# laboroai/border

Measured on AMD Instinct MI355X. Metric: agent opt-steps/sec (DQN Atari 84x84x4, batch 256), higher is better.
Workload: dtype f32 (conv2 / conv3 forward: 3xbf16 operand split, 6 products)

## Files before the change

border_amd/csrc/dqn.hip:

```cpp
#include <algorithm>
#include <atomic>
#include <chrono>
#include <cmath>
#include <string>

#include "common.hpp"
#include "agent_base.hpp"
#include "igemm.hpp"
#include "conv1_bf16_img.hpp"
#include "cnn_layers.hpp"
#include "igemm_b3.hpp"
#include "act_small.hpp"
#include "dqn_rollback.hpp"

using namespace bdr;

namespace {

#ifndef BDR_TEAMS
#define BDR_TEAMS 2
#endif
#ifndef BDR_TEAMS_FWD_C3
#define BDR_TEAMS_FWD_C3 BDR_TEAMS
#endif
#ifndef BDR_TEAMS_DX_L1
#define BDR_TEAMS_DX_L1 BDR_TEAMS
#endif
#ifndef BDR_TEAMS_DX_C3
#define BDR_TEAMS_DX_C3 BDR_TEAMS
#endif
#ifndef BDR_TEAMS_FWD_L1
#define BDR_TEAMS_FWD_L1 1
#endif
#ifndef BDR_TEAMS_FWD_C2
#define BDR_TEAMS_FWD_C2 1
#endif
#ifndef BDR_TEAMS_DX_C2
#define BDR_TEAMS_DX_C2 1
#endif
#ifndef BDR_TAIL_OVERLAP
#define BDR_TAIL_OVERLAP 1
#endif
#ifndef BDR_DXC2_MERGED
#define BDR_DXC2_MERGED 2
#endif
#ifndef BDR_FWDC3_SHAPE
#define BDR_FWDC3_SHAPE 1, 2, 1, 1
#endif
using FwdC3D = FwdConvP<GeomC3, BDR_FWDC3_SHAPE>;
constexpr size_t PL2_U16 = (size_t)3 * 64 * 512, PL3_U16 = (size_t)3 * 64 * 576;
constexpr size_t CPL_W2 = 0, CPL_W3 = PL2_U16, CPL_U16 = PL2_U16 + PL3_U16;
__device__ __forceinline__ size_t cpl_index(int k, int n) { return ((size_t)(k >> 5) * 64 + n) * 32 + (k & 31); }

__device__ __forceinline__ void conv_plane_store(uint16_t* __restrict__ pl, int layer, int e, float x)
{
    uint16_t v[3];
    split3_rn(x, v);
    const size_t n = (size_t)(layer ? 576 : 512) * 64, o = cpl_index(e >> 6, e & 63);
    uint16_t* d = pl + (layer ? CPL_W3 : CPL_W2);
    d[o] = v[0]; d[n + o] = v[1]; d[2 * n + o] = v[2];
}

__global__ __launch_bounds__(256) void k_conv_planes(const float* __restrict__ w2, const float* __restrict__ w3, uint16_t* __restrict__ pl)
{
    const int i = blockIdx.x * 256 + threadIdx.x;
    if (i < 512 * 64) conv_plane_store(pl, 0, i, w2[i]);
    else if (i < 512 * 64 + 576 * 64) conv_plane_store(pl, 1, i - 512 * 64, w3[i - 512 * 64]);
}
#ifndef BDR_FWDC2_B3_SHAPE
#define BDR_FWDC2_B3_SHAPE 2, 2
#endif
#ifndef BDR_FWDC3_B3_SHAPE
#define BDR_FWDC3_B3_SHAPE 2, 2
#endif
struct FwdB3Args : FwdArgs { const uint16_t* wpl[MAXZ]; };
template <class G, int WM_, int WN_, int TM_ = 1, int TN_ = 1>
struct FwdB3 : FwdP<G, AFwd<G>, WM_, WN_, false, 0, TM_, TN_> {
    using Args = FwdB3Args;
    __device__ static const uint4* b_chunk(const Args& a, int z, int, int pl, int kt, int n, int kq)
    {
        return reinterpret_cast<const uint4*>(a.wpl[z] + (size_t)pl * G::COUT * G::K + cpl_index(kt * 32 + kq * 8, n));
    }
};
using FwdC2B3 = FwdB3<GeomC2, BDR_FWDC2_B3_SHAPE>;
using FwdC3B3 = FwdB3<GeomC3, BDR_FWDC3_B3_SHAPE>;
constexpr int TEAMS_FWD_C2 = BDR_TEAMS_FWD_C2, TEAMS_FWD_C3 = BDR_TEAMS_FWD_C3, TEAMS_FWD_L1 = BDR_TEAMS_FWD_L1, TEAMS_DX_L1 = BDR_TEAMS_DX_L1,
              TEAMS_DX_C3 = BDR_TEAMS_DX_C3, TEAMS_DX_C2 = BDR_TEAMS_DX_C2;

struct HeadArgs {
    const float* p1[MAXZ];
    const float* b4[MAXZ];
    const float* w5[MAXZ];
    const float* b5[MAXZ];
    float* h1[MAXZ];
    float* q[MAXZ];
    int B, A, S;
};

struct TdArgs {
    int double_dqn;
    const uint8_t* act;
    int act_bytes;
    const float* reward;
    const int8_t* term;
    float* dh1;
    float* dq;
    float* pred;
    float* tgt;
    float* loss_row;
    int B, A;
    float gamma;
    int loss_kind;
    const float* weight;
    float* td_abs;
    int has_clip; float clip_min, clip_max;
    unsigned* err;
    const float* q_tgt_mem;
    int z_tgt, z_sel;
    unsigned* wait_sig; unsigned wait_epoch; unsigned long long wait_limit; unsigned* sig_err;
};

constexpr int HEAD_ROWS = 2;
template <int S, int AMAX>
__global__ __launch_bounds__(64 * HEAD_ROWS * MAXZ) void k_head(HeadArgs a, TdArgs t, int nz, int td)
{
    __shared__ float sq[HEAD_ROWS][MAXZ][64];
    const int lane = threadIdx.x & 63, wave = __builtin_amdgcn_readfirstlane(threadIdx.x >> 6);
    const int r = wave / nz, z = wave % nz;
    const int row = blockIdx.x * HEAD_ROWS + r;
    const bool valid = row < a.B;
    const int rw = valid ? row : 0;
    const int A = a.A;
    f32x4 part[S][2];
#pragma unroll
    for (int s = 0; s < S; ++s) {
        const float* p = a.p1[z] + ((size_t)s * a.B + rw) * 512 + lane * 8;
        part[s][0] = *reinterpret_cast<const f32x4*>(p);
        part[s][1] = *reinterpret_cast<const f32x4*>(p + 4);
    }
    const f32x4 b4lo = *reinterpret_cast<const f32x4*>(a.b4[z] + lane * 8), b4hi = *reinterpret_cast<const f32x4*>(a.b4[z] + lane * 8 + 4);
    const float* w5 = a.w5[z] + lane * 8;
    float wreg[8][AMAX];
#pragma unroll
    for (int k = 0; k < AMAX; ++k) {
        const float* wk = w5 + (size_t)min(k, A - 1) * 512;
        const f32x4 lo = *reinterpret_cast<const f32x4*>(wk), hi = *reinterpret_cast<const f32x4*>(wk + 4);
#pragma unroll
        for (int j = 0; j < 4; ++j) { wreg[j][k] = lo[j]; wreg[4 + j][k] = hi[j]; }
    }
    const float b5 = lane < A ? a.b5[z][lane] : 0.f;
    long long act = 0; float reward = 0.f, wgt = 1.f; int term = 0;
    if (td && z == 0) {
        act = *reinterpret_cast<const long long*>(t.act + (size_t)rw * t.act_bytes);
        if (act < 0 || act >= A) {
            if (lane == 0 && t.err) atomicOr(t.err + bdr_agent::ERR_ACTION, 1u);
            act = act < 0 ? 0 : A - 1;
        }
        reward = t.reward[rw]; term = (int)t.term[rw];
        if (t.weight) wgt = t.weight[rw];
    }

    f32x4 h[2] = {f32x4{0, 0, 0, 0}, f32x4{0, 0, 0, 0}};
#pragma unroll
    for (int s = 0; s < S; ++s) { h[0] += part[s][0]; h[1] += part[s][1]; }
    float hv[8];
#pragma unroll
    for (int j = 0; j < 8; ++j) {
        const float v = h[j >> 2][j & 3] + (j < 4 ? b4lo[j & 3] : b4hi[j & 3]);
        hv[j] = v > 0.f ? v : 0.f;
    }
    asm volatile("" ::"v"(act), "v"(reward), "v"(term), "v"(wgt), "v"(b5));
    if (valid) {
        float* ho = a.h1[z] + (size_t)row * 512 + lane * 8;
        *reinterpret_cast<f32x4*>(ho) = f32x4{hv[0], hv[1], hv[2], hv[3]};
        *reinterpret_cast<f32x4*>(ho + 4) = f32x4{hv[4], hv[5], hv[6], hv[7]};
    }
    float sk[AMAX];
#pragma unroll
    for (int k = 0; k < AMAX; ++k) {
        float s = 0.f;
#pragma unroll
        for (int j = 0; j < 8; ++j) s = fmaf(hv[j], wreg[j][k], s);
        sk[k] = s;
    }
#pragma unroll
    for (int off = 32; off > 0; off >>= 1)
#pragma unroll
        for (int k = 0; k < AMAX; ++k) sk[k] += __shfl_xor(sk[k], off);
    float qv = 0.f;
#pragma unroll
    for (int k = 0; k < AMAX; ++k) qv = lane == k ? sk[k] : qv;
    qv += b5;
    if (lane < A) {
        if (valid) a.q[z][(size_t)row * A + lane] = qv;
        sq[r][z][lane] = qv;
    }
    if (!td) return;
    if (t.q_tgt_mem && t.wait_sig) {
        if (threadIdx.x == 0) {
            const unsigned long long t0 = wall_clock64();
            while ((int)(__hip_atomic_load(t.wait_sig, __ATOMIC_ACQUIRE, __HIP_MEMORY_SCOPE_AGENT) - t.wait_epoch) < 0) {
                __builtin_amdgcn_s_sleep(2);
                if (__hip_atomic_load(t.sig_err, __ATOMIC_RELAXED, __HIP_MEMORY_SCOPE_AGENT) != 0) break;
                if (wall_clock64() - t0 > t.wait_limit) {
                    __hip_atomic_store(t.sig_err, 100u, __ATOMIC_RELAXED, __HIP_MEMORY_SCOPE_AGENT);
                    if (t.err) __hip_atomic_store(t.err + bdr_agent::ERR_GATE, 100u, __ATOMIC_RELAXED, __HIP_MEMORY_SCOPE_AGENT);
                    break;
                }
            }
        }
    }
    __syncthreads();
    if (z != 0 || !valid) return;
    if (t.q_tgt_mem) {
        __builtin_amdgcn_fence(__ATOMIC_ACQUIRE, "agent");
        if (lane < A) sq[r][MAXZ - 1][lane] = __builtin_nontemporal_load(t.q_tgt_mem + (size_t)row * A + lane);
    }
    const float* q_tg = t.q_tgt_mem ? sq[r][MAXZ - 1] : sq[r][t.z_tgt];
    const float* sel = t.z_sel >= 0 ? sq[r][t.z_sel] : q_tg;
    float v = lane < A ? sel[lane] : -INFINITY;
    int idx = lane;
#pragma unroll
    for (int off = 32; off > 0; off >>= 1) {
        const float ov = __shfl_xor(v, off);
        const int oi = __shfl_xor(idx, off);
        if (ov > v || (ov == v && oi < idx)) { v = ov; idx = oi; }
    }
    const float qn = q_tg[idx];
    const float pred = sq[r][0][act];
    const float tgt = td_target(reward, (float)(1 - term), t.gamma, qn);
    const TdLossIn li{t.loss_kind, t.weight != nullptr, wgt, t.has_clip, t.clip_min, t.clip_max};
    float lossb, tdv;
    const float dl = td_loss_row(pred, tgt, li, lossb, tdv);
    const float dq = dl / (float)a.B;
    if (lane == 0) {
        t.dq[row] = dq; t.pred[row] = pred; t.tgt[row] = tgt; t.loss_row[row] = lossb;
        if (t.td_abs) t.td_abs[row] = tdv;
    }
// ... 196 lines not shown
    BDR_TRY(alloc_f(&a->a1_alt, (size_t)B * 400 * 32));
    BDR_TRY(alloc_f(&a->dh1, (size_t)B * 512));
    BDR_TRY(alloc_f(&a->dy3, (size_t)B * 49 * 64));
    BDR_TRY(alloc_f(&a->dy2, (size_t)B * 81 * 64));
    BDR_TRY(alloc_f(&a->dy1, (size_t)B * 400 * 32));
    BDR_TRY(alloc_f(&a->dq, B)); BDR_TRY(alloc_f(&a->pred, B)); BDR_TRY(alloc_f(&a->tgt, B));
    BDR_TRY(alloc_f(&a->loss_row, B));
    const DwPlan p = dw_plan(B, a->ar.ns);
    BDR_TRY(alloc_f(&a->part, p.total));
    a->part_floats = p.total;
    a->B = B;
    return BDR_OK;
}

struct ConvReduceAdamArgs {
    Reduce3Args r;
    float* p; const float* g; float* m; float* v;
    float* gbase;
    size_t rest0_4, n4;
    AdamScalars s;
    int reduce_blocks;
    const unsigned* poison;
    int reduce_only;
    unsigned long long* applied; unsigned long long step;
    unsigned long long* applied2;
    int wg_base;
    uint16_t* cpl;
};
constexpr int SIG_HEAD = 0, SIG_DXL1 = 1, SIG_DXC3 = 2, SIG_SIDE = 3, SIG_GATHER = 4, SIG_TEST = 5, SIG_TEST_ERR = 6, SIG_ERR = 7, SIG_TGT = 8, SIG_TRACK = 9, SIG_MAIN_END = 10, SIG_XCONV = 11, SIG_XFC = 14;
constexpr int SIG_DXC2 = 15, SIG_CONV23 = SIG_SIDE;
__global__ __launch_bounds__(64) void k_gate(unsigned* sig, int which, unsigned epoch, unsigned long long* waited, int publish,
                                             unsigned long long limit = 1000000000ull , int err_slot = SIG_ERR,
                                             unsigned* dev_err = nullptr)
{
    if (threadIdx.x != 0) return;
    if (publish >= 0) __hip_atomic_store(sig + publish, epoch, __ATOMIC_RELAXED, __HIP_MEMORY_SCOPE_AGENT);
    if (err_slot == SIG_ERR && __hip_atomic_load(sig + SIG_ERR, __ATOMIC_RELAXED, __HIP_MEMORY_SCOPE_AGENT) != 0) return;
    const unsigned long long t0 = wall_clock64();
    while ((int)(__hip_atomic_load(sig + which, __ATOMIC_ACQUIRE, __HIP_MEMORY_SCOPE_AGENT) - epoch) < 0) {
        __builtin_amdgcn_s_sleep(4);
        if (wall_clock64() - t0 > limit || (err_slot == SIG_ERR && __hip_atomic_load(sig + SIG_ERR, __ATOMIC_RELAXED, __HIP_MEMORY_SCOPE_AGENT) != 0)) {
            __hip_atomic_store(sig + err_slot, 1u + (unsigned)which, __ATOMIC_RELAXED, __HIP_MEMORY_SCOPE_AGENT);
            if (dev_err) __hip_atomic_store(dev_err + bdr_agent::ERR_GATE, 1u + (unsigned)which, __ATOMIC_RELAXED, __HIP_MEMORY_SCOPE_AGENT);
            return;
        }
    }
    if (waited) {
        const unsigned long long dt = wall_clock64() - t0;
        waited[0] += dt; waited[1] += 1;
        unsigned long long* mx = waited + 22 - (which == SIG_SIDE ? 4 : which);
        if (dt > *mx) *mx = dt;
        if (which == SIG_SIDE) {
            const unsigned long long ts = *reinterpret_cast<volatile unsigned long long*>(sig + 12);
            if (ts && t0 > ts) waited[12] += t0 - ts;
        }
    }
}
__global__ __launch_bounds__(64) void k_signal(unsigned* sig, int which, unsigned epoch)
{
    if (threadIdx.x == 0 && which == SIG_SIDE) *reinterpret_cast<volatile unsigned long long*>(sig + 12) = wall_clock64();
    if (threadIdx.x == 0) __hip_atomic_store(sig + which, epoch, __ATOMIC_RELAXED, __HIP_MEMORY_SCOPE_AGENT);
}

__global__ void k_copy_word_unless(unsigned long long* dst, const unsigned long long* src, const unsigned* poison) { if (!(poison && *poison)) *dst = *src; }

__global__ __launch_bounds__(256) void k_reduce_adam(ConvReduceAdamArgs a)
{
    const bool poisoned = a.reduce_only || (a.poison && *a.poison != 0);
    if (a.applied && !poisoned && blockIdx.x == 0 && threadIdx.x == 0) { *a.applied = a.step; if (a.applied2) *a.applied2 = a.step; }
    if ((int)blockIdx.x >= a.reduce_blocks) {
        if (poisoned) return;
        const size_t i = a.rest0_4 + (size_t)(blockIdx.x - a.reduce_blocks) * 256 + threadIdx.x;
        if (i >= a.n4) return;
        f32x4 pp = reinterpret_cast<f32x4*>(a.p)[i], gg = reinterpret_cast<const f32x4*>(a.g)[i];
        f32x4 mm = reinterpret_cast<f32x4*>(a.m)[i], vv = reinterpret_cast<f32x4*>(a.v)[i];
#pragma unroll
        for (int j = 0; j < 4; ++j) {
            float pe = pp[j], me = mm[j], ve = vv[j];
            adam_element(pe, gg[j], me, ve, a.s);
            pp[j] = pe; mm[j] = me; vv[j] = ve;
        }
        reinterpret_cast<f32x4*>(a.p)[i] = pp;
        reinterpret_cast<f32x4*>(a.m)[i] = mm;
        reinterpret_cast<f32x4*>(a.v)[i] = vv;
        return;
    }
    __shared__ float red[8][32];
    const int bx = (int)blockIdx.x + a.wg_base;
    const int s_id = bx >= a.r.seg[2].wg0 ? 2 : (bx >= a.r.seg[1].wg0 ? 1 : 0);
    const ReduceSeg& sg = a.r.seg[s_id];
    const int o = threadIdx.x & 31, grp = threadIdx.x >> 5;
    const int i = (bx - sg.wg0) * 32 + o;
    float s = 0.f;
    if (i < sg.n) {
        int c = grp;
        for (; c + 24 < sg.chunks; c += 32) {
            const float v0 = sg.part[(size_t)c * sg.stride + i], v1 = sg.part[(size_t)(c + 8) * sg.stride + i];
            const float v2 = sg.part[(size_t)(c + 16) * sg.stride + i], v3 = sg.part[(size_t)(c + 24) * sg.stride + i];
            s += v0; s += v1; s += v2; s += v3;
        }
        for (; c < sg.chunks; c += 8) s += sg.part[(size_t)c * sg.stride + i];
    }
    red[grp][o] = s;
    __syncthreads();
    if (grp == 0 && i < sg.n) {
        float t = red[0][o];
#pragma unroll
        for (int k = 1; k < 8; ++k) t += red[k][o];
        const float g = i < sg.n_weights ? t * sg.wscale : t;
        sg.g[i] = g;
        if (poisoned) return;
        const size_t e = (size_t)(sg.g - a.gbase) + i;
        float pe = a.p[e], me = a.m[e], ve = a.v[e];
        adam_element(pe, g, me, ve, a.s);
        a.p[e] = pe; a.m[e] = me; a.v[e] = ve;
        if (a.cpl && s_id >= 1 && i < sg.n_weights) conv_plane_store(a.cpl, s_id - 1, i, pe);
    }
}

int effective_sched(DqnCnn* a);

struct NetInst { const uint8_t* x; const float* params; int slot; };

int32_t forward(DqnCnn* a, const NetInst* inst, int nz, int B, const TdArgs* td = nullptr, hipStream_t st = nullptr)
{
    if (!st) st = a->stream;
    const Arena& ar = a->ar;
    FwdArgs f{};
    bool uses_q = false;
    for (int z = 0; z < nz; ++z) uses_q = uses_q || inst[z].params == a->q;
    if (uses_q) BDR_TRY(a->join_exchange(true, false));
    {
        Conv1Args c{};
        c.M = B * 400; c.nz = nz;
        for (int z = 0; z < nz; ++z) {
            c.x[z] = inst[z].x; c.w1[z] = inst[z].params + ar.w1; c.bias[z] = inst[z].params + ar.b1; c.out[z] = a->a1[inst[z].slot];
        }
        Bracket br(a, "fwd_conv1");
        BDR_HIP(conv1_forward(ar.ns, B, st, c));
    }
    if (uses_q && st == a->stream) BDR_TRY(a->join_conv23());
    f.M = B * 81;
    for (int z = 0; z < nz; ++z) { f.x[z] = a->a1[inst[z].slot]; f.w[z] = inst[z].params + ar.w2; f.bias[z] = inst[z].params + ar.b2; f.out[z] = a->a2[inst[z].slot]; }
    bool b3 = a->conv_b3;
    FwdB3Args fb{};
    for (int z = 0; z < nz && b3; ++z) b3 = inst[z].params == a->q || inst[z].params == a->q_tgt;
    for (int z = 0; z < nz && b3; ++z) {
        const int set = inst[z].params == a->q ? 0 : 1;
        if (a->cpl_fresh[set] && !a->cpl_escaped[set]) continue;
        hipLaunchKernelGGL(k_conv_planes, dim3((512 * 64 + 576 * 64 + 255) / 256), dim3(256), 0, st, inst[z].params + ar.w2, inst[z].params + ar.w3, a->cpl[set]);
        BDR_HIP(hipGetLastError());
        a->cpl_fresh[set] = true;
    }
    if (b3) {
        static_cast<FwdArgs&>(fb) = f;
        for (int z = 0; z < nz; ++z) fb.wpl[z] = a->cpl[inst[z].params == a->q ? 0 : 1] + CPL_W2;
        Bracket br(a, "fwd_conv2");
        BDR_HIP((launch_igemm_b3<FwdC2B3, 6>(st, dim3(m_tiles<FwdC2B3>(f.M) * n_tiles<FwdC2B3>(), 1, nz), fb)));
    } else { Bracket br(a, "fwd_conv2"); BDR_HIP((launch_igemm<FwdC2, TEAMS_FWD_C2>(st, dim3(m_tiles<FwdC2>(f.M) * n_tiles<FwdC2>(), 1, nz), f))); }
    f.M = B * 49;
    for (int z = 0; z < nz; ++z) { f.x[z] = a->a2[inst[z].slot]; f.w[z] = inst[z].params + ar.w3; f.bias[z] = inst[z].params + ar.b3; f.out[z] = a->a3[inst[z].slot]; }
    if (b3) {
        static_cast<FwdArgs&>(fb) = f;
        for (int z = 0; z < nz; ++z) fb.wpl[z] = a->cpl[inst[z].params == a->q ? 0 : 1] + CPL_W3;
        Bracket br(a, "fwd_conv3");
        BDR_HIP((launch_igemm_b3<FwdC3B3, 6>(st, dim3(m_tiles<FwdC3B3>(f.M) * n_tiles<FwdC3B3>(), 1, nz), fb)));
    } else { Bracket br(a, "fwd_conv3"); BDR_HIP((launch_igemm<FwdC3D, TEAMS_FWD_C3>(st, dim3(m_tiles<FwdC3D>(f.M) * n_tiles<FwdC3D>(), 1, nz), f))); }
    f.M = B; f.nkt_per_split = (98 + L1_SPLIT - 1) / L1_SPLIT;
    for (int z = 0; z < nz; ++z) { f.x[z] = a->a3[inst[z].slot]; f.w[z] = inst[z].params + ar.w4; f.bias[z] = nullptr; f.out[z] = a->p1[inst[z].slot]; }
    if (uses_q) BDR_TRY(a->join_exchange(false, true));
    {
        Bracket br(a, "fwd_l1");
#if BDR_L1_XSPLIT
        static_assert(L1_SPLIT == 8, "FwdL1X: one k-slice per XCD");
        BDR_HIP((launch_igemm<FwdL1X, TEAMS_FWD_L1>(st, dim3(m_tiles<FwdL1X>(B) * n_tiles<FwdL1X>() * 8, 1, nz), f)));
#else
        if (nz % 2 == 0) BDR_HIP((launch_igemm<FwdL1Z2, TEAMS_FWD_L1>(st, dim3(((B + 63) / 64) * 16, L1_SPLIT, nz / 2), f)));
        else BDR_HIP((launch_igemm<FwdL1, TEAMS_FWD_L1>(st, dim3(((B + 63) / 64) * 8, L1_SPLIT, nz), f)));
#endif
    }
    HeadArgs h{};
    h.B = B; h.A = ar.A; h.S = L1_SPLIT;
    for (int z = 0; z < nz; ++z) {
        h.p1[z] = a->p1[inst[z].slot]; h.b4[z] = inst[z].params + ar.b4; h.w5[z] = inst[z].params + ar.w5;
        h.b5[z] = inst[z].params + ar.b5; h.h1[z] = a->h1[inst[z].slot]; h.q[z] = a->qv[inst[z].slot];
    }
    {
        Bracket br(a, td ? "head_fwd_td" : "head_fwd");
        const dim3 grid((B + HEAD_ROWS - 1) / HEAD_ROWS), block(64 * HEAD_ROWS * nz);
        const TdArgs tv = td ? *td : TdArgs{};
        hipEvent_t stop = td && effective_sched(a) == 1 && a->kev ? a->ev_fork[0] : nullptr;
        const int tdi = td ? 1 : 0;
        if (ar.A <= 8) hipExtLaunchKernelGGL((k_head<L1_SPLIT, 8>), grid, block, 0, st, nullptr, stop, 0, h, tv, nz, tdi);
        else if (ar.A <= 24) hipExtLaunchKernelGGL((k_head<L1_SPLIT, 24>), grid, block, 0, st, nullptr, stop, 0, h, tv, nz, tdi);
        else hipExtLaunchKernelGGL((k_head<L1_SPLIT, 64>), grid, block, 0, st, nullptr, stop, 0, h, tv, nz, tdi);
        BDR_HIP(hipGetLastError());
    }
    return BDR_OK;
}

AdamScalars adam_scalars(const bdr_dqn_config& c, uint64_t step)
{
    return adam_scalars_for(c.opt_kind == BDR_OPT_ADAMW, c.lr, c.beta1, c.beta2, c.eps, c.weight_decay, step);
}

int32_t launch_gate(DqnCnn* a, hipStream_t st, int which, unsigned epoch, int publish)
{
    unsigned long long* tr = a->gate_trace && which <= SIG_SIDE ? a->gate_trace + 2 * (st == a->stream ? 4 : which) : nullptr;
    hipLaunchKernelGGL(k_gate, dim3(1), dim3(64), 0, st, a->sig, which, epoch, tr, publish, a->gate_limit, SIG_ERR, a->dev_err);
    BDR_HIP(hipGetLastError());
    return BDR_OK;
}

int32_t queues_independent(DqnCnn* a, hipStream_t waiter, hipStream_t producer, bool* ok)
{
    a->test_epoch += 1;
    BDR_HIP(hipMemsetAsync(a->sig + SIG_TEST_ERR, 0, sizeof(unsigned), waiter));
    hipLaunchKernelGGL(k_gate, dim3(1), dim3(64), 0, waiter, a->sig, SIG_TEST, a->test_epoch, (unsigned long long*)nullptr, -1, 10000000ull, SIG_TEST_ERR,
                       (unsigned*)nullptr);
    BDR_HIP(hipGetLastError());
    hipLaunchKernelGGL(k_signal, dim3(1), dim3(64), 0, producer, a->sig, SIG_TEST, a->test_epoch);
    BDR_HIP(hipGetLastError());
    BDR_HIP(hipStreamSynchronize(waiter));
    BDR_HIP(hipStreamSynchronize(producer));
    unsigned err = 0;
    BDR_HIP(hipMemcpy(&err, a->sig + SIG_TEST_ERR, sizeof err, hipMemcpyDeviceToHost));
    *ok = err == 0;
    return BDR_OK;
}

std::atomic<DqnCnn*> g_gate_owner{nullptr};
bool claim_gates(DqnCnn* a)
{
    if (a->holds_gate_token) return true;
    DqnCnn* expected = nullptr;
    if (g_gate_owner.compare_exchange_strong(expected, a)) { a->holds_gate_token = true; return true; }
    return false;
}
int effective_sched(DqnCnn* a)
{
    if (a->prof) return 0;
    if (a->sched == 3 && !claim_gates(a)) {
        if (!a->noted_event_fallback) {
            a->noted_event_fallback = true;
            fprintf(stderr, "border_amd: another DQN agent of this process already orders its two queues with device flags; this agent orders its "
                            "queues with events (same results, ~10 %% slower steps) for as long as that agent lives\n");
        }
        return 1;
    }
    return a->sched;
}

int32_t update_critic(DqnCnn* a, int B, const uint8_t* obs, const uint8_t* next_obs, const uint8_t* act, int act_bytes,
                      const float* reward, const int8_t* term, const float* weight = nullptr, bdr_replay* per_buffer = nullptr)
{
    BDR_TRY(ensure_batch(a, B));
    BDR_TRY(a->td_buffer(B));
    a->last_reward = reward; a->last_B = B;
    const Arena& ar = a->ar;
    const bdr_dqn_config& c = a->cfg;
    if (a->conv23_join_pending) std::swap(a->a1[0], a->a1_alt);
    NetInst inst[3] = {{obs, a->q, 0}, {next_obs, a->q_tgt, 1}, {next_obs, a->q, 2}};

    TdArgs t{};
    t.double_dqn = c.double_dqn;
    t.act = act; t.act_bytes = act_bytes; t.reward = reward; t.term = term;
    t.dh1 = a->dh1; t.dq = a->dq; t.pred = a->pred; t.tgt = a->tgt;
    t.loss_row = a->loss_row; t.B = B; t.A = ar.A; t.gamma = (float)c.discount_factor; t.loss_kind = c.critic_loss;
    t.weight = weight; t.td_abs = a->td_abs;
    t.has_clip = c.has_clip_td_err; t.clip_min = (float)c.clip_td_err_min; t.clip_max = (float)c.clip_td_err_max;
    t.err = a->dev_err;
    t.z_tgt = 1; t.z_sel = c.double_dqn ? 2 : -1;
    if (a->tgt_enqueued) {
        a->tgt_enqueued = false;
        NetInst on[2] = {{obs, a->q, 0}, {next_obs, a->q, 2}};
        t.q_tgt_mem = a->qv[1]; t.z_tgt = -1; t.z_sel = c.double_dqn ? 1 : -1;
        t.wait_sig = a->sig + SIG_TGT; t.wait_epoch = a->sig_epoch + 1; t.wait_limit = a->gate_limit; t.sig_err = a->sig + SIG_ERR;
        BDR_TRY(forward(a, on, c.double_dqn ? 2 : 1, B, &t));
    } else {
        BDR_TRY(forward(a, inst, c.double_dqn ? 3 : 2, B, &t));
    }

    const int sched = effective_sched(a);
    const bool ov = sched == 1;
    const bool gated = sched == 3;
    hipStream_t sd = ov || gated ? a->side : a->stream;
    const unsigned epoch = gated ? ++a->sig_epoch : 0;
    auto sigf = [&](int which) -> unsigned* { return gated ? a->sig + which : nullptr; };
    auto gate = [&](hipStream_t st, int which) -> int32_t { return launch_gate(a, st, which, epoch, -1); };
    const unsigned any = sched == 2 ? hipExtAnyOrderLaunch : 0;
    auto kev = [&](int k) -> hipEvent_t { return ov && a->kev ? a->ev_fork[k] : nullptr; };
    auto fork = [&](int k) -> int32_t {
        if (!ov) return BDR_OK;
        if (!a->kev) BDR_HIP(hipEventRecord(a->ev_fork[k], a->stream));
        BDR_HIP(hipStreamWaitEvent(a->side, a->ev_fork[k], 0));
        return BDR_OK;
    };
    const DwPlan pl = dw_plan(a->B, ar.ns);
    const bool defer = a->defer_adam;
    const bool tail = gated && BDR_TAIL_OVERLAP != 0 && !defer;
    if (!defer) a->adam_step += 1;
    const AdamScalars adam_s = adam_scalars(c, std::max<uint64_t>(a->adam_step, 1));

    auto head_bwd = [&]() -> int32_t {
        HeadBwdArgs hb{a->h1[0], a->dq, act, act_bytes, a->loss_row, a->grad + ar.w5, a->grad + ar.b5, a->loss, B, ar.A};
        Bracket br(a, "head_bwd");
        LAUNCH_FL(sd, any, nullptr, k_head_bwd, dim3(2 * ar.A + 1), dim3(256), hb);
        return BDR_OK;
    };
    auto l1_dw = [&]() -> int32_t {
        DwArgs d{a->a3[0], a->dh1, a->grad + ar.w4, 0, B};
        Bracket br(a, "bwd_l1_dw");
        LAUNCH_FL(sd, any, nullptr, k_igemm_red<DwL1>, dim3(49 * 8), dim3(256), d);
        return BDR_OK;
    };
    auto l1_dx = [&]() -> int32_t {
        DxArgs d{a->dh1, a->q + ar.w4, a->a3[0], a->dy3, B, sigf(SIG_HEAD), epoch};
        Bracket br(a, "bwd_l1_dx");
        BDR_HIP((launch_igemm<DxL1, TEAMS_DX_L1>(a->stream, dim3((m_tiles<DxL1>(B) * n_tiles<DxL1>() + 7) / 8 * 8, 1, 1), d, 0, kev(1))));
        return BDR_OK;
// ... 785 lines not shown
```

Baseline: 5296.

## Fuse conv2 and conv3 forward into one per-image 3xbf16 kernel

Adds a fused kernel that runs conv2 and conv3 for one image per workgroup. The conv1 activation is split into three bf16 planes in LDS, conv2 output is produced and kept in LDS as split planes, and conv3 consumes it directly, with double-buffered weight staging. It still writes a2 for the backward pass but removes one kernel launch and the global round trip between the two layers. The trade-off is a grid of only B*nz workgroups at one wave per EU using most of the LDS, and some waves sit idle during the conv2 phase. The fused path is taken only when not profiling and, by default, only on the main stream.

```diff
diff --git a/border_amd/csrc/dqn.hip b/border_amd/csrc/dqn.hip
--- a/border_amd/csrc/dqn.hip
+++ b/border_amd/csrc/dqn.hip
@@ -10,6 +10,7 @@
 #include "conv1_bf16_img.hpp"
 #include "cnn_layers.hpp"
 #include "igemm_b3.hpp"
+#include "fwd_c23_b3.hpp"
 #include "act_small.hpp"
 #include "dqn_rollback.hpp"
 
@@ -48,42 +49,9 @@
 #define BDR_FWDC3_SHAPE 1, 2, 1, 1
 #endif
 using FwdC3D = FwdConvP<GeomC3, BDR_FWDC3_SHAPE>;
-constexpr size_t PL2_U16 = (size_t)3 * 64 * 512, PL3_U16 = (size_t)3 * 64 * 576;
-constexpr size_t CPL_W2 = 0, CPL_W3 = PL2_U16, CPL_U16 = PL2_U16 + PL3_U16;
-__device__ __forceinline__ size_t cpl_index(int k, int n) { return ((size_t)(k >> 5) * 64 + n) * 32 + (k & 31); }
-
-__device__ __forceinline__ void conv_plane_store(uint16_t* __restrict__ pl, int layer, int e, float x)
-{
-    uint16_t v[3];
-    split3_rn(x, v);
-    const size_t n = (size_t)(layer ? 576 : 512) * 64, o = cpl_index(e >> 6, e & 63);
-    uint16_t* d = pl + (layer ? CPL_W3 : CPL_W2);
-    d[o] = v[0]; d[n + o] = v[1]; d[2 * n + o] = v[2];
-}
-
-__global__ __launch_bounds__(256) void k_conv_planes(const float* __restrict__ w2, const float* __restrict__ w3, uint16_t* __restrict__ pl)
-{
-    const int i = blockIdx.x * 256 + threadIdx.x;
-    if (i < 512 * 64) conv_plane_store(pl, 0, i, w2[i]);
-    else if (i < 512 * 64 + 576 * 64) conv_plane_store(pl, 1, i - 512 * 64, w3[i - 512 * 64]);
-}
-#ifndef BDR_FWDC2_B3_SHAPE
-#define BDR_FWDC2_B3_SHAPE 2, 2
+#ifndef BDR_FUSED_CONV23
+#define BDR_FUSED_CONV23 1
 #endif
-#ifndef BDR_FWDC3_B3_SHAPE
-#define BDR_FWDC3_B3_SHAPE 2, 2
-#endif
-struct FwdB3Args : FwdArgs { const uint16_t* wpl[MAXZ]; };
-template <class G, int WM_, int WN_, int TM_ = 1, int TN_ = 1>
-struct FwdB3 : FwdP<G, AFwd<G>, WM_, WN_, false, 0, TM_, TN_> {
-    using Args = FwdB3Args;
-    __device__ static const uint4* b_chunk(const Args& a, int z, int, int pl, int kt, int n, int kq)
-    {
-        return reinterpret_cast<const uint4*>(a.wpl[z] + (size_t)pl * G::COUT * G::K + cpl_index(kt * 32 + kq * 8, n));
-    }
-};
-using FwdC2B3 = FwdB3<GeomC2, BDR_FWDC2_B3_SHAPE>;
-using FwdC3B3 = FwdB3<GeomC3, BDR_FWDC3_B3_SHAPE>;
 constexpr int TEAMS_FWD_C2 = BDR_TEAMS_FWD_C2, TEAMS_FWD_C3 = BDR_TEAMS_FWD_C3, TEAMS_FWD_L1 = BDR_TEAMS_FWD_L1, TEAMS_DX_L1 = BDR_TEAMS_DX_L1,
               TEAMS_DX_C3 = BDR_TEAMS_DX_C3, TEAMS_DX_C2 = BDR_TEAMS_DX_C2;
 
@@ -586,20 +554,30 @@
         BDR_HIP(hipGetLastError());
         a->cpl_fresh[set] = true;
     }
-    if (b3) {
-        static_cast<FwdArgs&>(fb) = f;
-        for (int z = 0; z < nz; ++z) fb.wpl[z] = a->cpl[inst[z].params == a->q ? 0 : 1] + CPL_W2;
-        Bracket br(a, "fwd_conv2");
-        BDR_HIP((launch_igemm_b3<FwdC2B3, 6>(st, dim3(m_tiles<FwdC2B3>(f.M) * n_tiles<FwdC2B3>(), 1, nz), fb)));
-    } else { Bracket br(a, "fwd_conv2"); BDR_HIP((launch_igemm<FwdC2, TEAMS_FWD_C2>(st, dim3(m_tiles<FwdC2>(f.M) * n_tiles<FwdC2>(), 1, nz), f))); }
-    f.M = B * 49;
-    for (int z = 0; z < nz; ++z) { f.x[z] = a->a2[inst[z].slot]; f.w[z] = inst[z].params + ar.w3; f.bias[z] = inst[z].params + ar.b3; f.out[z] = a->a3[inst[z].slot]; }
-    if (b3) {
-        static_cast<FwdArgs&>(fb) = f;
-        for (int z = 0; z < nz; ++z) fb.wpl[z] = a->cpl[inst[z].params == a->q ? 0 : 1] + CPL_W3;
-        Bracket br(a, "fwd_conv3");
-        BDR_HIP((launch_igemm_b3<FwdC3B3, 6>(st, dim3(m_tiles<FwdC3B3>(f.M) * n_tiles<FwdC3B3>(), 1, nz), fb)));
-    } else { Bracket br(a, "fwd_conv3"); BDR_HIP((launch_igemm<FwdC3D, TEAMS_FWD_C3>(st, dim3(m_tiles<FwdC3D>(f.M) * n_tiles<FwdC3D>(), 1, nz), f))); }
+    if (b3 && BDR_FUSED_CONV23 != 0 && !a->prof && (BDR_FUSED_CONV23 == 2 || st == a->stream)) {
+        FwdC23Args c{};
+        for (int z = 0; z < nz; ++z) {
+            c.a1[z] = a->a1[inst[z].slot]; c.cpl[z] = a->cpl[inst[z].params == a->q ? 0 : 1];
+            c.b2[z] = inst[z].params + ar.b2; c.b3[z] = inst[z].params + ar.b3;
+            c.a2[z] = a->a2[inst[z].slot]; c.a3[z] = a->a3[inst[z].slot];
+        }
+        BDR_HIP(launch_fwd_c23_b3(st, B, nz, c));
+    } else {
+        if (b3) {
+            static_cast<FwdArgs&>(fb) = f;
+            for (int z = 0; z < nz; ++z) fb.wpl[z] = a->cpl[inst[z].params == a->q ? 0 : 1] + CPL_W2;
+            Bracket br(a, "fwd_conv2");
+            BDR_HIP((launch_igemm_b3<FwdC2B3, 6>(st, dim3(m_tiles<FwdC2B3>(f.M) * n_tiles<FwdC2B3>(), 1, nz), fb)));
+        } else { Bracket br(a, "fwd_conv2"); BDR_HIP((launch_igemm<FwdC2, TEAMS_FWD_C2>(st, dim3(m_tiles<FwdC2>(f.M) * n_tiles<FwdC2>(), 1, nz), f))); }
+        f.M = B * 49;
+        for (int z = 0; z < nz; ++z) { f.x[z] = a->a2[inst[z].slot]; f.w[z] = inst[z].params + ar.w3; f.bias[z] = inst[z].params + ar.b3; f.out[z] = a->a3[inst[z].slot]; }
+        if (b3) {
+            static_cast<FwdArgs&>(fb) = f;
+            for (int z = 0; z < nz; ++z) fb.wpl[z] = a->cpl[inst[z].params == a->q ? 0 : 1] + CPL_W3;
+            Bracket br(a, "fwd_conv3");
+            BDR_HIP((launch_igemm_b3<FwdC3B3, 6>(st, dim3(m_tiles<FwdC3B3>(f.M) * n_tiles<FwdC3B3>(), 1, nz), fb)));
+        } else { Bracket br(a, "fwd_conv3"); BDR_HIP((launch_igemm<FwdC3D, TEAMS_FWD_C3>(st, dim3(m_tiles<FwdC3D>(f.M) * n_tiles<FwdC3D>(), 1, nz), f))); }
+    }
     f.M = B; f.nkt_per_split = (98 + L1_SPLIT - 1) / L1_SPLIT;
     for (int z = 0; z < nz; ++z) { f.x[z] = a->a3[inst[z].slot]; f.w[z] = inst[z].params + ar.w4; f.bias[z] = nullptr; f.out[z] = a->p1[inst[z].slot]; }
     if (uses_q) BDR_TRY(a->join_exchange(false, true));
diff --git a/border_amd/csrc/fwd_c23_b3.hpp b/border_amd/csrc/fwd_c23_b3.hpp
--- /dev/null
+++ b/border_amd/csrc/fwd_c23_b3.hpp
@@ -0,0 +1,237 @@
+#pragma once
+#include "cnn_layers.hpp"
+#include "igemm_b3.hpp"
+
+namespace {
+
+constexpr size_t PL2_U16 = (size_t)3 * 64 * 512, PL3_U16 = (size_t)3 * 64 * 576;
+constexpr size_t CPL_W2 = 0, CPL_W3 = PL2_U16, CPL_U16 = PL2_U16 + PL3_U16;
+__device__ __forceinline__ size_t cpl_index(int k, int n) { return ((size_t)(k >> 5) * 64 + n) * 32 + (k & 31); }
+
+__device__ __forceinline__ void conv_plane_store(uint16_t* __restrict__ pl, int layer, int e, float x)
+{
+    uint16_t v[3];
+    split3_rn(x, v);
+    const size_t n = (size_t)(layer ? 576 : 512) * 64, o = cpl_index(e >> 6, e & 63);
+    uint16_t* d = pl + (layer ? CPL_W3 : CPL_W2);
+    d[o] = v[0]; d[n + o] = v[1]; d[2 * n + o] = v[2];
+}
+
+__global__ __launch_bounds__(256) void k_conv_planes(const float* __restrict__ w2, const float* __restrict__ w3, uint16_t* __restrict__ pl)
+{
+    const int i = blockIdx.x * 256 + threadIdx.x;
+    if (i < 512 * 64) conv_plane_store(pl, 0, i, w2[i]);
+    else if (i < 512 * 64 + 576 * 64) conv_plane_store(pl, 1, i - 512 * 64, w3[i - 512 * 64]);
+}
+#ifndef BDR_FWDC2_B3_SHAPE
+#define BDR_FWDC2_B3_SHAPE 2, 2
+#endif
+#ifndef BDR_FWDC3_B3_SHAPE
+#define BDR_FWDC3_B3_SHAPE 2, 2
+#endif
+struct FwdB3Args : FwdArgs { const uint16_t* wpl[MAXZ]; };
+template <class G, int WM_, int WN_, int TM_ = 1, int TN_ = 1>
+struct FwdB3 : FwdP<G, AFwd<G>, WM_, WN_, false, 0, TM_, TN_> {
+    using Args = FwdB3Args;
+    __device__ static const uint4* b_chunk(const Args& a, int z, int, int pl, int kt, int n, int kq)
+    {
+        return reinterpret_cast<const uint4*>(a.wpl[z] + (size_t)pl * G::COUT * G::K + cpl_index(kt * 32 + kq * 8, n));
+    }
+};
+using FwdC2B3 = FwdB3<GeomC2, BDR_FWDC2_B3_SHAPE>;
+using FwdC3B3 = FwdB3<GeomC3, BDR_FWDC3_B3_SHAPE>;
+
+struct FwdC23Args {
+    const float* a1[MAXZ];
+    const uint16_t* cpl[MAXZ];
+    const float* b2[MAXZ];
+    const float* b3[MAXZ];
+    float* a2[MAXZ];
+    float* a3[MAXZ];
+};
+
+constexpr int C23_A1_BLK = 108;
+constexpr int C23_PL_A1 = 4 * C23_A1_BLK * 32;
+constexpr int C23_A2_PIX = 84;
+constexpr int C23_PL_A2 = C23_A2_PIX * 64;
+constexpr int C23_PL_W = 64 * B3_ROW, C23_W_STAGE = 3 * C23_PL_W;
+constexpr int C23_NKT2 = GeomC2::K / BK, C23_NKT3 = GeomC3::K / BK, C23_NKT = C23_NKT2 + C23_NKT3;
+constexpr int C23_LDS_U16 = 3 * C23_PL_A1 + 3 * C23_PL_A2 + 2 * C23_W_STAGE;
+static_assert(C23_LDS_U16 * 2 <= 160 * 1024, "one workgroup per CU");
+static_assert(C23_NKT2 % 2 == 0 && C23_NKT3 % 2 == 0, "the k loops are unrolled by two (stage and register set of a tile = its parity)");
+__device__ __forceinline__ int c23_a1_off(int P, int c) { return P * 32 + ((c ^ ((P >> 2) & 3)) << 3); }
+__device__ __forceinline__ int c23_a2_off(int P, int c) { return P * 64 + ((c ^ ((P >> 1) & 7)) << 3); }
+
+static __global__ __launch_bounds__(256) __attribute__((amdgpu_waves_per_eu(1, 1))) void k_fwd_c23_b3(FwdC23Args a)
+{
+    __shared__ __attribute__((aligned(16))) uint16_t smem[C23_LDS_U16];
+    uint16_t* const sA1 = smem;
+    uint16_t* const sA2 = sA1 + 3 * C23_PL_A1;
+    uint16_t* const sW = sA2 + 3 * C23_PL_A2;
+    const int tid = threadIdx.x, lane = tid & 63, wave = __builtin_amdgcn_readfirstlane(tid >> 6);
+    const int j = lane & 31, h = lane >> 5;
+    const int img = blockIdx.x, z = blockIdx.z;
+    using Set0 = std::integral_constant<int, 0>;
+    using Set1 = std::integral_constant<int, 1>;
+    using One = std::integral_constant<int, 1>;
+    using Two = std::integral_constant<int, 2>;
+
+    const uint16_t* const w2 = a.cpl[z] + CPL_W2 + tid * 8;
+    const uint16_t* const w3 = a.cpl[z] + CPL_W3 + tid * 8;
+    u32x4_t rb[2][3];
+    auto wload = [&](auto set, int g) {
+        constexpr int S = decltype(set)::value;
+        g = min(g, C23_NKT - 1);
+        const bool l2 = g < C23_NKT2;
+        const uint16_t* p = l2 ? w2 + (size_t)g * C23_PL_W : w3 + (size_t)(g - C23_NKT2) * C23_PL_W;
+        const size_t ps = l2 ? (size_t)64 * GeomC2::K : (size_t)64 * GeomC3::K;
+#pragma unroll
+        for (int pl = 0; pl < 3; ++pl) rb[S][pl] = *reinterpret_cast<const u32x4_t*>(p + pl * ps);
+    };
+    const int w_off = b3_off(tid >> 2, tid & 3);
+    auto wcommit = [&](auto set, int stage) {
+        constexpr int S = decltype(set)::value;
+#pragma unroll
+        for (int pl = 0; pl < 3; ++pl) *reinterpret_cast<u32x4_t*>(&sW[stage * C23_W_STAGE + pl * C23_PL_W + w_off]) = rb[S][pl];
+    };
+
+    constexpr int A1_V4 = 400 * 32 / 4, A1_PASSES = (A1_V4 + 255) / 256;
+    f32x4 st[A1_PASSES];
+    {
+        const f32x4* src = reinterpret_cast<const f32x4*>(a.a1[z] + (size_t)img * (400 * 32));
+#pragma unroll
+        for (int p = 0; p < A1_PASSES; ++p) st[p] = src[min(tid + 256 * p, A1_V4 - 1)];
+    }
+    wload(Set0{}, 0);
+    wload(Set1{}, 1);
+    f32x4 bq2[2][4], bq3[4];
+#pragma unroll
+    for (int q = 0; q < 4; ++q) {
+        bq2[0][q] = *reinterpret_cast<const f32x4*>(a.b2[z] + 8 * q + 4 * h);
+        bq2[1][q] = *reinterpret_cast<const f32x4*>(a.b2[z] + 32 + 8 * q + 4 * h);
+        bq3[q] = *reinterpret_cast<const f32x4*>(a.b3[z] + 32 * (wave & 1) + 8 * q + 4 * h);
+    }
+#pragma unroll
+    for (int p = 0; p < A1_PASSES; ++p) {
+        const int i = tid + 256 * p;
+        if (A1_V4 % 256 != 0 && i >= A1_V4) continue;
+        const int pix = i >> 3, q4 = i & 7, ih = pix / 20, iw = pix - 20 * ih;
+        const int P = ((ih & 1) * 2 + (iw & 1)) * C23_A1_BLK + (ih >> 1) * 10 + (iw >> 1);
+        u32x2_t sp[3];
+        split3_f32x4(st[p], sp);
+        const int o = c23_a1_off(P, q4 >> 1) + (q4 & 1) * 4;
+#pragma unroll
+        for (int pl = 0; pl < 3; ++pl) *reinterpret_cast<u32x2_t*>(&sA1[pl * C23_PL_A1 + o]) = sp[pl];
+    }
+    wcommit(Set0{}, 0);
+    wload(Set0{}, 2);
+    __syncthreads();
+
+    f32x16 acc[2];
+    bf16x8_t fx[2][3], fw[2][2][3];
+    auto load_frag = [&](auto buf, auto tn_, const uint16_t* sX, int plx, int xoff, int stage, int s, int ct0) {
+        constexpr int F = decltype(buf)::value, TN = decltype(tn_)::value;
+#pragma unroll
+        for (int pl = 0; pl < 3; ++pl) {
+            fx[F][pl] = *reinterpret_cast<const bf16x8_t*>(&sX[pl * plx + xoff]);
+#pragma unroll
+            for (int tn = 0; tn < TN; ++tn)
+                fw[F][tn][pl] = *reinterpret_cast<const bf16x8_t*>(&sW[stage * C23_W_STAGE + pl * C23_PL_W + b3_off((ct0 + tn) * 32 + j, s * 2 + h)]);
+        }
+    };
+    auto mfma6 = [&](auto buf, auto tn_) {
+        constexpr int F = decltype(buf)::value, TN = decltype(tn_)::value;
+        constexpr int ORD[6][2] = {{2, 0}, {0, 2}, {1, 1}, {1, 0}, {0, 1}, {0, 0}};
+#pragma unroll
+        for (int t = 0; t < 6; ++t)
+#pragma unroll
+            for (int tn = 0; tn < TN; ++tn)
+                acc[tn] = __builtin_amdgcn_mfma_f32_32x32x16_bf16(fw[F][tn][ORD[t][1]], fx[F][ORD[t][0]], acc[tn], 0, 0, 0);
+    };
+    auto tile = [&](auto par, auto tn_, const uint16_t* sX, int plx, auto&& xoff, int T0, int kt, int nkt, bool active, int ct0) {
+        constexpr int PAR = decltype(par)::value;
+        using SetN = std::integral_constant<int, PAR ^ 1>;
+        const int g = T0 + kt;
+        if (active) load_frag(Set1{}, tn_, sX, plx, xoff(kt, 1), PAR, 1, ct0);
+        if (g + 1 < C23_NKT) wcommit(SetN{}, PAR ^ 1);
+        wload(SetN{}, g + 3);
+        if (active) mfma6(Set0{}, tn_);
+        __builtin_amdgcn_sched_barrier(0);
+        __syncthreads();
+        if (active && kt + 1 < nkt) load_frag(Set0{}, tn_, sX, plx, xoff(kt + 1, 0), PAR ^ 1, 0, ct0);
+        if (active) mfma6(Set1{}, tn_);
+        __builtin_amdgcn_sched_barrier(0);
+    };
+
+    {
+        const bool active = wave < 3;
+        const int v = min(wave, 2) * 32 + j;
+        auto xoff = [&](int kt, int s) {
+            const int kh = kt >> 2, kw = kt & 3;
+            return c23_a1_off(((kh & 1) * 2 + (kw & 1)) * C23_A1_BLK + v + 10 * (kh >> 1) + (kw >> 1), 2 * s + h);
+        };
+#pragma unroll
+        for (int tn = 0; tn < 2; ++tn)
+#pragma unroll
+            for (int r = 0; r < 16; ++r) acc[tn][r] = 0.f;
+        if (active) load_frag(Set0{}, Two{}, sA1, C23_PL_A1, xoff(0, 0), 0, 0, 0);
+        for (int kt = 0; kt < C23_NKT2; kt += 2) {
+            tile(Set0{}, Two{}, sA1, C23_PL_A1, xoff, 0, kt, C23_NKT2, active, 0);
+            tile(Set1{}, Two{}, sA1, C23_PL_A1, xoff, 0, kt + 1, C23_NKT2, active, 0);
+        }
+        const int oh = v / 10, ow = v - 10 * oh;
+        if (active && oh < 9 && ow < 9) {
+            const int m = oh * 9 + ow;
+            float* out = a.a2[z] + ((size_t)img * 81 + m) * 64 + 4 * h;
+#pragma unroll
+            for (int tn = 0; tn < 2; ++tn)
+#pragma unroll
+                for (int q = 0; q < 4; ++q) {
+                    f32x4 y;
+#pragma unroll
+                    for (int e = 0; e < 4; ++e) { const float t = acc[tn][4 * q + e] + bq2[tn][q][e]; y[e] = t > 0.f ? t : 0.f; }
+                    *reinterpret_cast<f32x4*>(out + 32 * tn + 8 * q) = y;
+                    u32x2_t sp[3];
+                    split3_f32x4(y, sp);
+                    const int o = c23_a2_off(m, 4 * tn + q) + 4 * h;
+#pragma unroll
+                    for (int pl = 0; pl < 3; ++pl) *reinterpret_cast<u32x2_t*>(&sA2[pl * C23_PL_A2 + o]) = sp[pl];
+                }
+        }
+    }
+    __syncthreads();
+
+    {
+        const int v = (wave >> 1) * 32 + j, ct = wave & 1;
+        auto xoff = [&](int kt, int s) {
+            const int tap = kt >> 1, kh = tap / 3, kw = tap - 3 * kh;
+            return c23_a2_off(v + 9 * kh + kw, (kt & 1) * 4 + 2 * s + h);
+        };
+#pragma unroll
+        for (int r = 0; r < 16; ++r) acc[0][r] = 0.f;
+        load_frag(Set0{}, One{}, sA2, C23_PL_A2, xoff(0, 0), 0, 0, ct);
+        for (int kt = 0; kt < C23_NKT3; kt += 2) {
+            tile(Set0{}, One{}, sA2, C23_PL_A2, xoff, C23_NKT2, kt, C23_NKT3, true, ct);
+            tile(Set1{}, One{}, sA2, C23_PL_A2, xoff, C23_NKT2, kt + 1, C23_NKT3, true, ct);
+        }
+        const int oh = v / 9, ow = v - 9 * oh;
+        if (oh < 7 && ow < 7) {
+            float* out = a.a3[z] + ((size_t)img * 49 + oh * 7 + ow) * 64 + 32 * ct + 4 * h;
+#pragma unroll
+            for (int q = 0; q < 4; ++q) {
+                f32x4 y;
+#pragma unroll
+                for (int e = 0; e < 4; ++e) { const float t = acc[0][4 * q + e] + bq3[q][e]; y[e] = t > 0.f ? t : 0.f; }
+                *reinterpret_cast<f32x4*>(out + 8 * q) = y;
+            }
+        }
+    }
+}
+
+inline hipError_t launch_fwd_c23_b3(hipStream_t st, int B, int nz, const FwdC23Args& args)
+{
+    hipLaunchKernelGGL(k_fwd_c23_b3, dim3(B, 1, nz), dim3(256), 0, st, args);
+    return hipGetLastError();
+}
+
+}
```

Result: faster. 5538 (median of 6 runs) (+4.6%).
